# BriansIDP/espnet_slurp

Measured on AMD Instinct MI355X. Metric: utterances/sec (fbank80x1500, Conformer-12L CTC+attn), higher is better.
Workload: dtype f32; 1 GPU; C2 SLURP Conformer-medium d=256 H=4 FF=1024 12L enc / 6L dec, V=600, rel_pos=latest, ctc 0.3, lsm 0.1, dropout 0.1, SpecAug on; global_batch=384, seq_len=1500, parallelism=dp1

## Files before the change

### espnet_slurp_amd/_native.py

```python
from __future__ import annotations

import ctypes
import os

_HERE = os.path.dirname(os.path.abspath(__file__))
LIB_PATH = os.path.join(_HERE, "libespnet_mi355%s.so" % os.environ.get("ESP_LIB_VARIANT", ""))

P = ctypes.c_void_p
I = ctypes.c_int
L = ctypes.c_long
F = ctypes.c_float
U64 = ctypes.c_ulonglong

SIGNATURES = {
    "esp_last_error": [],
    "esp_abi_version": [],
    "esp_gemm_bf16": [I, I, I, I, I, I, I, P, L, L, L, P, L, L, L, P, L, L, L, P, F, F, P, I, P, F, U64, I, P, P, P, L,
                      P],
    "esp_gemm_bf16_pl": [I, I, I, I, I, I, I, P, L, L, L, P, L, L, L, P, L, L, L, P, F, F, I, P, F, U64, I, P, I,
                         L, P, L, P],
    "esp_f32_to_bf16": [P, P, L, I, L, L, I, P],
    "esp_conv2_fwd_bf16": [P, P, P, P, I, I, I, I, P, L, P],
    "esp_conv2_dgrad_bf16": [P, P, P, P, I, I, I, I, P, P, L, P],
    "esp_conv1_fwd_bf16": [P, P, P, P, P, I, I, I, I, P],
# ... 43 lines not shown
    "esp_csgu_bwd_norm": [P, P, P, P, P, P, L, I, P, I, I, I, P, P],
    "esp_bn_swish_fwd": [P, P, P, P, P, P, P, P, F, F, I, I, P, L, I, P, P],
    "esp_bn_swish_eval": [P, P, P, P, P, P, F, I, I, P, P, P],
    "esp_bn_swish_fwd_planes": [P, P, P, P, L, L, I, P, P, P, P, F, F, I, I, P, L, I, P, P],
    "esp_bn_swish_bwd": [P, P, P, P, P, P, P, P, P, I, I, P, L, P, I, P, P],
    "esp_heads_split": [P, L, I, I, I, I, I, P, P, P],
    "esp_heads_split2": [P, L, I, I, I, I, I, P, P, P, P, P],
    "esp_add2d": [P, L, P, L, I, I, P],
    "esp_attn_softmax_fwd": [P, P, I, I, F, P, I, I, P, P, F, U64, I, I, I, L, L, P, P],
    "esp_attn_softmax_bwd": [P, P, P, F, U64, F, L, I, L, P],
    "esp_relshift_bwd": [P, L, P, L, I, I, I, I, P],
    "esp_relpos_attn_fwd": [P, P, P, L, P, L, I, I, F, P, P, P, F, U64, I, L, P],
    "esp_relpos_attn_probs": [P, P, P, L, P, L, I, I, I, F, P, P, P, F, U64, I, L, P, P],
    "esp_attn_bwd_prep": [P, L, P, L, I, I, I, I, P, P, L, I, P],
    "esp_attn_dscores": [P, L, P, L, P, P, P, P, L, I, I, I, I, F, F, U64, I, L, P],
    "esp_attn_softmax_bwd_relpos": [P, P, P, P, L, I, F, U64, F, L, I, L, P, P],
    "esp_attn_softmax_bwd_relpos_band": [P, P, P, P, L, F, U64, F, L, I, L, P],
    "esp_relpos_dqv": [P, L, P, L, P, L, I, I, I, P, L, P],
    "esp_relpos_dq": [P, L, P, L, P, L, P, L, P, I, I, I, P],
    "esp_relpos_attn_bwd": [P, L, P, L, P, P, P, L, I, I, F, F, U64, I, L, P],
    "esp_relpos_flash_fwd": [P, P, P, L, P, L, P, L, I, I, I, F, P, P, L, P, F, U64, I, P],
    "esp_relpos_flash_bwd": [P, P, P, L, P, L, P, L, I, I, I, F, P, P, P, L, P, F, U64, I, P, L, P, P, L, P, P, P],
    "esp_relpos_dp": [P, L, P, I, I, I, I, P, L, P, P, P, P, P, L, P, L, P],
    "esp_fbank_fwd": [P, L, P, I, I, I, I, P, P, P, P, P, I, P, I, P, P],
    "esp_global_mvn": [P, P, I, I, I, P, P, I, I, P],
    "esp_conv2_dgrad": [P, P, P, P, I, I, I, I, P, P, L, P],
    "esp_conv1_fwd": [P, P, P, P, I, I, I, I, P],
    "esp_conv1_fwd_bits": [P, P, P, P, P, P, I, I, I, I, P],
    "esp_conv2_dgrad_bits": [P, P, P, P, P, I, I, I, I, P, P, L, P],
    "esp_conv2_dgrad_c1fold": [P, P, P, P, P, I, I, P, P, I, I, I, I, P, P, L, P, L, P],
# ... 28 lines not shown
    "esp_cbt_unchunk_bwd": [P, P, I, I, I, I, I, I, I, P],
    "esp_conv1_dgrad": [P, P, P, I, I, I, I, P],
    "esp_grad_norm_workspace_bytes": [L],
    "esp_layernorm_bwd_workspace_bytes": [I, I],
    "esp_colsum_workspace_bytes": [I, I],
    "esp_dwconv1d_wgrad_workspace_bytes": [I, I, I, I],
    "esp_bn_swish_fwd_workspace_bytes": [I, I],
    "esp_bn_swish_bwd_workspace_bytes": [I, I],
    "esp_conv1_wgrad_workspace_bytes": [I, I, I, I],
    "esp_conv2_dgrad_workspace_bytes": [I],
    "esp_ctc_loss_workspace_bytes": [I, I, I],
    "esp_relpos_dp_workspace_bytes": [I, I, I],
}
_RESTYPES = {"esp_last_error": ctypes.c_char_p, "esp_abi_version": I, "esp_attn_slot_check_errors": I, "esp_set_gemm_compute": I,
             "esp_get_gemm_compute": I, "esp_set_splitk_mode": I, "esp_set_wgrad_ws": I,
             "esp_f32_gemm_products": I}
_RESTYPES.update({k: L for k in SIGNATURES if k.endswith("_workspace_bytes")})
ABI_VERSION = 39

_lib = None


def load() -> ctypes.CDLL:
    global _lib
    if _lib is not None:
        return _lib
    if not os.path.exists(LIB_PATH):
        raise RuntimeError(
            f"espnet_slurp_amd: native library not found at {LIB_PATH}; "
            "build it with `make -C espnet_slurp_amd/csrc` (no CPU fallback exists)")
    lib = ctypes.CDLL(LIB_PATH)
    for name, args in SIGNATURES.items():
        fn = getattr(lib, name)
# ... 28 lines not shown
```

### espnet_slurp_amd/blocks.py

```python
from __future__ import annotations

import math
from typing import List, Optional

import torch
from torch import nn

from . import kernels as K


def _mix64(x: int) -> int:
    x &= 0xFFFFFFFFFFFFFFFF
    x = ((x ^ (x >> 30)) * 0xBF58476D1CE4E5B9) & 0xFFFFFFFFFFFFFFFF
    x = ((x ^ (x >> 27)) * 0x94D049BB133111EB) & 0xFFFFFFFFFFFFFFFF
    return x ^ (x >> 31)


class Seeds:

    def __init__(self, base: int):
        self.base = base & 0xFFFFFFFFFFFFFFFF
        self.i = 0

    def next(self) -> int:
# ... 273 lines not shown
                   batch=Z, nb2=B, sa=(B * T * Pp, T * Pp), sb=(dk, 0), sc=(dk, T * D))
        K.colsum(tmp, self.pos_bias_v.grad.view(-1), accumulate=True)
        K.add2d(tmp, D, dqkv, 3 * D, M, D)
        dp = empty(P, D, like=dctx)
        K.gemm(P, dk, B * T, dbd, c.q_v, dp, mode_a=K.RC, lda=Pp, mode_b=K.RC, ldb=dk, ldc=D,
               batch=H, nb2=1, sa=(B * T * Pp, 0), sb=(B * T * dk, 0), sc=(dk, 0))
        return dp

    def _bwd_ds(self, c, dctx, dqkv):
        H, dk = self.h, self.d_k
        D = H * dk
        B, T, P = c.B, c.T, c.P
        Z = H * B
        Tp = K.pitch(T)
        dS = empty(Z * T * Tp, like=dctx)
        dot = empty(Z * T, like=dctx)
        K.attn_bwd_prep(dctx, D, c.ctx, D, B, H, dk, T, dot, None, 0, 1)
        K.attn_dscores(dctx, D, c.qkv, 3 * D, c.attn, dot, dS, None, 0, 1, B, H, dk, math.sqrt(dk), c.pa, c.sa, T,
                       Tp, v_off=2 * D)
        self._dv(c, c.pv, dctx, dqkv)
        bias_part = empty(Z * ((T + 31) // 32) * 2 * dk, like=dctx)
        K.relpos_dq(dS, Tp, c.qkv, 3 * D, c.p, D, dqkv, 3 * D, bias_part, B, H, T, k_off=D)
        self._dk(c, dS, dqkv)
        dp = empty(P, D, like=dctx)
        K.relpos_dp(dS, Tp, c.q_v, 1, B, H, T, dp, D, bias_part, None, self.pos_bias_u.grad.view(-1),
                    self.pos_bias_v.grad.view(-1), dqkv, 3 * D)
        return dp

    def _bwd_flash(self, c, dctx, dqkv):
        H, dk = self.h, self.d_k
        D = H * dk
        B, T, P = c.B, c.T, c.P
        Z = H * B
        rel = 2 if self.legacy else 1
# ... 467 lines not shown
```

### espnet_slurp_amd/csrc/attention.hip

```cpp
#include <stdlib.h>

#include <type_traits>

#include "common.h"

namespace {

constexpr int RP_ROWS = 32, RP_DK = 64;

__global__ void heads_split_kernel(const float* __restrict__ src, long ld, int col0, int B, int T, int H, int dk,
                                   const float* __restrict__ bias, float* __restrict__ dst) {
  const long n = (long)H * B * T * dk;
  for (long i = blockIdx.x * (long)blockDim.x + threadIdx.x; i < n; i += (long)gridDim.x * blockDim.x) {
    const int d = (int)(i % dk);
    long r = i / dk;
    const int t = (int)(r % T);
    r /= T;
    const int b = (int)(r % B);
    const int h = (int)(r / B);
    float v = src[((long)b * T + t) * ld + col0 + h * dk + d];
    if (bias) v += bias[h * dk + d];
    dst[i] = v;
  }
}
// ... 660 lines not shown
  for (int t = 0; t < NTA; ++t) {
    const int j = (wave + 4 * t) * 32 + l32;
    if (j >= T) continue;
#pragma unroll
    for (int r = 0; r < 16; ++r) {
      const int i = i0 + (r & 3) + 8 * (r >> 2) + 4 * hf;
      if (i >= T) continue;
      const long row = (long)z * T + i;
      const float pe = sc[t][r] * sm[r];
      attn[row * lds + j] = pe;
      if (pdrop) pdrop[row * lds + j] = esp::keep_elem(seed, (uint64_t)(row * T + j), thr) ? pe * dscale : 0.f;
    }
  }
}

typedef __attribute__((ext_vector_type(8))) __bf16 attn_bf16x8;
struct Frag16 {
  attn_bf16x8 v[2];
};
__device__ __forceinline__ void split_frag(const float (&f)[16], Frag16& o) {
#pragma unroll
  for (int m = 0; m < 2; ++m) {
    uint32_t h[4];
#pragma unroll
    for (int j = 0; j < 4; ++j) h[j] = esp::bf16_pair(f[8 * m + 2 * j], f[8 * m + 2 * j + 1]);
    o.v[m] = __builtin_bit_cast(attn_bf16x8, make_uint4(h[0], h[1], h[2], h[3]));
  }
}
__device__ __forceinline__ f32x4 mfma_np(const Frag16& a, const Frag16& b, f32x4 c) {
#pragma unroll
  for (int m = 0; m < 2; ++m) c = __builtin_amdgcn_mfma_f32_16x16x32_bf16(a.v[m], b.v[m], c, 0, 0, 0);
  return c;
}

#ifndef ESP_ATTN_PROBS_LDS
#define ESP_ATTN_PROBS_LDS 1
#endif
#ifndef ESP_ATTN_PREFETCH
#define ESP_ATTN_PREFETCH 3
#endif

constexpr int RW_ROWS = 16, RW_PITCH = 37;
constexpr int RW_SPITCH = 64;
__device__ __forceinline__ void keep_quad(uint64_t seed, uint64_t ix, uint32_t thr, bool even_T, bool idx32, bool& k0,
                                          bool& k1, bool& k2, bool& k3) {
  if (even_T && idx32) {
    esp::keep_pair32(seed, (uint32_t)ix, thr, k0, k1);
    esp::keep_pair32(seed, (uint32_t)ix + 2, thr, k2, k3);
  } else if (even_T) {
    esp::keep_pair(seed, ix, thr, k0, k1);
    esp::keep_pair(seed, ix + 2, thr, k2, k3);
  } else {
    k0 = esp::keep_elem(seed, ix, thr);
    k1 = esp::keep_elem(seed, ix + 1, thr);
    k2 = esp::keep_elem(seed, ix + 2, thr);
    k3 = esp::keep_elem(seed, ix + 3, thr);
  }
}
template <int NTA, bool P2, bool LEGACY, int SPLIT = 1, int XS = 0>
__global__ __launch_bounds__(256, 2) void relpos_attn_fwd16_kernel(
    const float* __restrict__ qu, const float* __restrict__ qv, const float* __restrict__ kmat, long ldk,
    const float* __restrict__ pm, long ldpm, int nb, float sqrt_dk, const int* __restrict__ klen,
    float* __restrict__ attn, float* __restrict__ pdrop, uint32_t thr, float dscale, uint64_t seed, int T, long lds,
    const uint64_t* __restrict__ key, const int* __restrict__ tvalid, int nrb, int Z) {
  __shared__ float ring[4][RW_ROWS * RW_PITCH];
  __shared__ __attribute__((aligned(16))) float stage[4][RW_ROWS * RW_SPITCH];
  __shared__ float xch[2][4][RW_ROWS];
  const int lane = threadIdx.x & 63, wave = threadIdx.x >> 6;
  const int xcd = blockIdx.x & 7, jb = blockIdx.x >> 3, zq = jb / nrb;
  const int z = zq * 8 + xcd, bx = jb - zq * nrb;
  if (z >= Z) return;
  const int i0 = (SPLIT == 1 ? bx * 4 + wave : bx * 2 + (wave >> 1)) * RW_ROWS;
  const int t0 = SPLIT == 1 ? 0 : (wave & 1) * NTA;
// ... 204 lines not shown
            d.x = k0 ? v.x * dscale : 0.f;
            d.y = k1 ? v.y * dscale : 0.f;
            d.z = k2 ? v.z * dscale : 0.f;
            d.w = k3 ? v.w * dscale : 0.f;
            *reinterpret_cast<float4*>(dbase[ps] + 16 * (t0 + t4)) = d;
          }
        }
      }
      asm volatile("" ::: "memory");
    }
  };
  if (pdrop) store_rows(std::true_type{});
  else store_rows(std::false_type{});
}

__device__ __forceinline__ int swz16(int r) { return ((r >> 1) & 1) | (r & 4); }
template <int NPL>
struct FragPl {
  attn_bf16x8 v[NPL][2];
};
template <int NPL>
__device__ __forceinline__ void split_row16(const float (&f)[16], FragPl<NPL>& o) {
#pragma unroll
  for (int m = 0; m < 2; ++m) {
    uint32_t h[4], md[4], l[4];
#pragma unroll
    for (int j = 0; j < 4; ++j) {
      if constexpr (NPL == 3) esp::split3_pair(f[8 * m + 2 * j], f[8 * m + 2 * j + 1], h[j], md[j], l[j]);
      else h[j] = esp::bf16_pair(f[8 * m + 2 * j], f[8 * m + 2 * j + 1]);
    }
    o.v[0][m] = __builtin_bit_cast(attn_bf16x8, make_uint4(h[0], h[1], h[2], h[3]));
    if constexpr (NPL == 3) {
      o.v[1][m] = __builtin_bit_cast(attn_bf16x8, make_uint4(md[0], md[1], md[2], md[3]));
      o.v[2][m] = __builtin_bit_cast(attn_bf16x8, make_uint4(l[0], l[1], l[2], l[3]));
    }
  }
}
template <int NPL>
__device__ __forceinline__ void read_frag_pl(const uint8_t* tile, int plane_bytes, int li, int q4, FragPl<NPL>& o) {
#pragma unroll
  for (int p = 0; p < NPL; ++p)
#pragma unroll
    for (int m = 0; m < 2; ++m)
      o.v[p][m] = *reinterpret_cast<const attn_bf16x8*>(tile + p * plane_bytes + li * 128 + (((2 * q4 + m) ^ swz16(li)) << 4));
}
template <int NPL>
__device__ __forceinline__ f32x4 mfma_pl(const FragPl<NPL>& a, const FragPl<NPL>& b, f32x4 c) {
#pragma unroll
  for (int m = 0; m < 2; ++m) {
    if constexpr (NPL == 3) {
      c = __builtin_amdgcn_mfma_f32_16x16x32_bf16(a.v[1][m], b.v[1][m], c, 0, 0, 0);
      c = __builtin_amdgcn_mfma_f32_16x16x32_bf16(a.v[2][m], b.v[0][m], c, 0, 0, 0);
      c = __builtin_amdgcn_mfma_f32_16x16x32_bf16(a.v[0][m], b.v[2][m], c, 0, 0, 0);
      c = __builtin_amdgcn_mfma_f32_16x16x32_bf16(a.v[1][m], b.v[0][m], c, 0, 0, 0);
      c = __builtin_amdgcn_mfma_f32_16x16x32_bf16(a.v[0][m], b.v[1][m], c, 0, 0, 0);
    }
    c = __builtin_amdgcn_mfma_f32_16x16x32_bf16(a.v[0][m], b.v[0][m], c, 0, 0, 0);
  }
  return c;
}

#ifndef ESP_ATTN_SLOT_CHECK
#define ESP_ATTN_SLOT_CHECK 0
#endif
#if ESP_ATTN_SLOT_CHECK
__device__ int g_attn_slot_err[64];
#endif
template <int NTA, bool P2, bool LEGACY, int NP>
__global__ __launch_bounds__(256, 2) void relpos_probs_lds_kernel(
    const float* __restrict__ qu, const float* __restrict__ qv, const float* __restrict__ kmat, long ldk,
    const float* __restrict__ pm, long ldpm, int nb, float sqrt_dk, const int* __restrict__ klen,
    float* __restrict__ attn, float* __restrict__ pdrop, uint32_t thr, float dscale, uint64_t seed, int T, long lds,
    const uint64_t* __restrict__ key, const int* __restrict__ tvalid, int nrb, int Z) {
  constexpr int NPL = NP == 6 ? 3 : 1;
  constexpr int PLB = RW_ROWS * 128;
// ... 31 lines not shown
    asm volatile("" ::: "memory");
    bool bad = false;
#pragma unroll
    for (int w = 0; w < 4; ++w) bad |= gw[w] != v;
    asm volatile("" ::: "memory");
    if (bad) g_attn_slot_err[lane] = 1 + where;
  };
#define ESP_SLOT_MARK(g, v) mark(g, v)
#define ESP_SLOT_CHECK(g, v, w) check(g, v, w)
#else
#define ESP_SLOT_MARK(g, v) ((void)0)
#define ESP_SLOT_CHECK(g, v, w) ((void)0)
#endif

  const int sr = tid >> 4, sd = 4 * (tid & 15);
  const int woff = sr * 128 + (((sd >> 3) ^ swz16(sr)) << 4) + ((sd >> 2) & 1) * 8;
  auto k_src = [&](int t) {
    return reinterpret_cast<const float4*>(kmat + ((long)b * T + min(t * 16 + sr, T - 1)) * ldk + head * RP_DK + sd);
  };
  auto p_src = [&](int u) {
    int pos = pbase + 16 * u + sr;
    if (LEGACY && pos > Ts) pos -= Ts + 1;
    return reinterpret_cast<const float4*>(pm + (long)min(max(pos, 0), P - 1) * ldpm + head * RP_DK + sd);
  };
  auto put_tile = [&](uint8_t* dst, const float4 v) {
    if constexpr (NPL == 3) {
      uint32_t h0, m0, l0, h1, m1, l1;
      esp::split3_pair(v.x, v.y, h0, m0, l0);
      esp::split3_pair(v.z, v.w, h1, m1, l1);
      *reinterpret_cast<uint2*>(dst + woff) = make_uint2(h0, h1);
      *reinterpret_cast<uint2*>(dst + PLB + woff) = make_uint2(m0, m1);
      *reinterpret_cast<uint2*>(dst + 2 * PLB + woff) = make_uint2(l0, l1);
    } else {
      *reinterpret_cast<uint2*>(dst + woff) = make_uint2(esp::bf16_pair(v.x, v.y), esp::bf16_pair(v.z, v.w));
    }
  };
  {
    float4 pv[PSL];
#pragma unroll
    for (int s = 0; s < PSL; ++s) pv[s] = *p_src(s - 4);
    const float4 kv = *k_src(0);
#pragma unroll
    for (int s = 0; s < PSL; ++s) {
      ESP_SLOT_MARK(pgen[pslot(s - 4)], BUSY);
      put_tile(ppl[pslot(s - 4)], pv[s]);
      ESP_SLOT_MARK(pgen[pslot(s - 4)], s - 4);
    }
    ESP_SLOT_MARK(kgen[0], BUSY);
    put_tile(kpl[0], kv);
    ESP_SLOT_MARK(kgen[0], 0);
    if constexpr (LEGACY) {
// ... 176 lines not shown
      }
      asm volatile("" ::: "memory");
    }
  };
  if (pdrop) store_rows(std::true_type{});
  else store_rows(std::false_type{});
#undef ESP_SLOT_MARK
#undef ESP_SLOT_CHECK
}

inline int gridn(long n) {
  long b = (n + 255) / 256;
  return (int)(b > 65536 ? 65536 : (b < 1 ? 1 : b));
}

template <int... Cs>
struct IntList {};
template <int C0, int... Cs, class F>
inline void dispatch_ge(IntList<C0, Cs...>, int v, F&& f) {
  if constexpr (sizeof...(Cs) == 0) {
    f(std::integral_constant<int, C0>{});
  } else {
    if (v <= C0) f(std::integral_constant<int, C0>{});
    else dispatch_ge(IntList<Cs...>{}, v, f);
  }
}
template <class F>
inline void dispatch_bool(bool b, F&& f) {
  if (b) f(std::true_type{});
  else f(std::false_type{});
}
struct DropArgs {
  uint32_t thr;
  float scale;
};
inline DropArgs drop_args(float drop_p) {
  const uint32_t thr = esp::drop_threshold(drop_p);
  return {thr, esp::drop_scale(thr)};
}
inline DropArgs drop_args(float drop_p, float*& pdrop) {
  const DropArgs d = drop_args(drop_p);
  if (!d.thr) pdrop = nullptr;
  return d;
}
inline bool is_pow2(float x) { return x > 0.f && (__builtin_bit_cast(uint32_t, x) & 0x7fffffu) == 0; }
using Per64 = IntList<1, 2, 4, 8, 16>;

}

ESP_API int esp_attn_slot_check_errors(void) {
#if ESP_ATTN_SLOT_CHECK
  if (hipDeviceSynchronize() != hipSuccess) return -2;
  int h[64];
  if (hipMemcpyFromSymbol(h, HIP_SYMBOL(g_attn_slot_err), sizeof h) != hipSuccess) return -2;
  int n = 0;
  for (int i = 0; i < 64; ++i) n += h[i] != 0;
  const int zeros[64] = {};
  if (hipMemcpyToSymbol(HIP_SYMBOL(g_attn_slot_err), zeros, sizeof zeros) != hipSuccess) return -2;
  return n;
// ... 295 lines not shown
```

### espnet_slurp_amd/csrc/attention_bwd.hip

```cpp
#include <stdlib.h>

#include "common.h"

namespace {

constexpr int QR = 32, QDK = 64, QKS = 32;
typedef __attribute__((ext_vector_type(8))) __bf16 bf16x8;

__device__ __forceinline__ int il_of(int r, int hf) { return (r & 3) + 8 * (r >> 2) + 4 * hf; }

__device__ __forceinline__ void split8(const float* v, bf16x8 (&o)[3]) {
  uint32_t H[4], M[4], L[4];
#pragma unroll
  for (int p = 0; p < 4; ++p) esp::split3_pair(v[2 * p], v[2 * p + 1], H[p], M[p], L[p]);
  o[0] = __builtin_bit_cast(bf16x8, make_uint4(H[0], H[1], H[2], H[3]));
  o[1] = __builtin_bit_cast(bf16x8, make_uint4(M[0], M[1], M[2], M[3]));
  o[2] = __builtin_bit_cast(bf16x8, make_uint4(L[0], L[1], L[2], L[3]));
}
__device__ __forceinline__ void mma6(f32x16& acc, const bf16x8 (&a)[3], const bf16x8 (&b)[3]) {
  constexpr int PA[6] = {1, 2, 0, 1, 0, 0}, PB[6] = {1, 0, 2, 0, 1, 0};
#pragma unroll
  for (int p = 0; p < 6; ++p) acc = __builtin_amdgcn_mfma_f32_32x32x16_bf16(a[PA[p]], b[PB[p]], acc, 0, 0, 0);
}

// ... 134 lines not shown
  if (job == 1) {
#pragma unroll
    for (int r = 0; r < 16; ++r) vt[(c * QR + il_of(r, hf)) * VP + l32] = acc[r];
  }
  __syncthreads();
  if (job == 0) {
#pragma unroll
    for (int r = 0; r < 16; ++r) {
      const int row = il_of(r, hf);
      if (i0 + row < T)
        dq[((long)b * T + i0 + row) * ldq + QDK * head + 32 * c + l32] = acc[r] + vt[(c * QR + row) * VP + l32];
    }
  }
}

}

static int relpos_dq_pitch(int T) { return (T + 31) / 32 * 32 + 4; }

ESP_API int esp_relpos_dq(const float* dS, long lds, const float* kmat, long ldk, const float* p, long ldpm, float* dq,
                          long ldq, float* bias_part, int nb, int H, int T, void* stream) {
  ESP_ARG_CHECK(T >= 1 && nb >= 1 && H >= 1 && lds >= T && lds % 4 == 0 && ((uintptr_t)dS & 15) == 0,
                "esp_relpos_dq: bad sizes T=%d lds=%ld (lds %% 4 == 0, dS 16-B aligned)", T, lds);
  const int DSP = relpos_dq_pitch(T);
  size_t shm = (size_t)QR * DSP * sizeof(float);
  if (shm < 2 * QR * 33 * sizeof(float)) shm = 2 * QR * 33 * sizeof(float);
  ESP_ARG_CHECK(shm <= 65536 && DSP <= 512, "esp_relpos_dq: T=%d needs %zu B of LDS (T <= 480)", T, shm);
  ESP_ARG_CHECK(dq && bias_part && kmat && p, "esp_relpos_dq: null operand");
  ESP_ARG_CHECK(ldk >= 64 && ldpm >= 64 && ldk < (1L << 22) && ldpm < (1L << 22) && 4L * T * ldk < (1L << 31) &&
                    4L * (2 * T - 1) * ldpm < (1L << 31),
// ... 8 lines not shown
```

### espnet_slurp_amd/csrc/elementwise.hip

```cpp
#include <stdarg.h>
#include <stdio.h>

#include "common.h"

namespace esp {
static thread_local char g_err[512] = "";
static const uint64_t* g_rng_key = nullptr;
const uint64_t* rng_key_ptr() { return g_rng_key; }
void set_error(const char* fmt, ...) {
  va_list ap;
  va_start(ap, fmt);
  vsnprintf(g_err, sizeof(g_err), fmt, ap);
  va_end(ap);
}
}

ESP_API const char* esp_last_error(void) { return esp::g_err; }
ESP_API int esp_abi_version(void) { return 39; }
ESP_API int esp_set_rng_key(const unsigned long long* key) {
  esp::g_rng_key = (const uint64_t*)key;
  return 0;
}

namespace {


inline int grid_for(long n, int per_thread = 1) {
  long b = (n / per_thread + 255) / 256;
  if (b > 65536) b = 65536;
  return (int)(b < 1 ? 1 : b);
}

__global__ void act_bwd_kernel(const float* __restrict__ dy, const float* __restrict__ h,
// ... 552 lines not shown
```

### espnet_slurp_amd/kernels.py

```python
from __future__ import annotations

import math
import os
from typing import Optional, Sequence

import torch

from . import _native

KC, RC, I2C_KC, I2C_RC = 0, 1, 2, 3
ACT_NONE, ACT_RELU, ACT_SWISH = 0, 1, 2
ACT_MUL = 3
ACT_AUX_DERIV = 16


def _p(t: Optional[torch.Tensor], off: int = 0):
    if t is None:
        return None
    return t.data_ptr() + off * t.element_size()


def _st():
    return torch.cuda.current_stream().cuda_stream

# ... 699 lines not shown
    lib = _native.load()
    prev = lib.esp_set_splitk_mode(int(mode))
    if prev < 0:
        raise _native.NativeError(f"esp_set_splitk_mode failed: {lib.esp_last_error().decode()}")
    return prev


def set_wgrad_ws(mode: int) -> int:
    lib = _native.load()
    prev = lib.esp_set_wgrad_ws(int(mode))
    if prev < 0:
        raise _native.NativeError(f"esp_set_wgrad_ws failed: {lib.esp_last_error().decode()}")
    return prev


def get_gemm_compute() -> int:
    return _native.load().esp_get_gemm_compute()


class gemm_compute:

    def __init__(self, dtype):
        self.dtype = dtype

    def __enter__(self):
        self.prev = set_gemm_compute(self.dtype)
        return self

    def __exit__(self, *exc):
        set_gemm_compute(self.prev)
# ... 185 lines not shown
def attn_dscores(dctx, ldd, vmat, ldv, attn, dot, dS, dbd, ldp, relpos, nb, H, dk, sqrt_dk, drop_p, seed, T, lds,
                 v_off=0):
    _f32(dctx, vmat, attn, dot, dS, dbd)
    if _PROF is not None:
        ev0 = torch.cuda.Event(enable_timing=True)
        ev1 = torch.cuda.Event(enable_timing=True)
        ev0.record()
    _native.call("esp_attn_dscores", _p(dctx), ldd, _p(vmat, v_off), ldv, _p(attn), _p(dot), _p(dS), _p(dbd), ldp,
                 int(relpos), nb, H, dk, float(sqrt_dk), float(drop_p), int(seed) & (2 ** 64 - 1), T, lds, _st())
    if _PROF is not None:
        ev1.record()
        _PROF.append((2.0 * T * T * dk * nb * H, ev0, ev1, (KC, KC, T, T, dk, nb * H, "dscores"),
                      (8.0 if dbd is not None else 4.0) * T * T * nb * H))


FLASH_ATTN = False
ATTN_FWD32 = False
FUSED_ATTN_BWD = False
ATTN_DSCORES = False
RELPOS_BWD_DS = True


def flash_ok(T: int, dk: int) -> bool:
    return FLASH_ATTN and dk == 64 and 1 <= T <= 512


def relpos_probs_ok(T: int, dk: int) -> bool:
    return dk == 64 and T <= 512


def relpos_fused_ok(T: int, dk: int) -> bool:
    return dk == 64 and (32 * (32 * ((T + 62) // 32) + 4) + 256) * 4 <= 65536


def relpos_bwd_ds_ok(T: int, dk: int) -> bool:
    return dk == 64 and 1 <= T <= 480 and pitch(T) % 4 == 0


def relpos_attn_paths(T: int, dk: int, legacy: bool, bucketed: bool):
    if flash_ok(T, dk) and not bucketed:
        fwd = "flash"
    elif relpos_probs_ok(T, dk) and not ATTN_FWD32:
        fwd = "probs"
    elif not legacy and relpos_fused_ok(T, dk):
        fwd = "block32"
    else:
        fwd = "gemm"
    if fwd == "flash":
        bwd = "flash"
    elif (not legacy and RELPOS_BWD_DS and relpos_bwd_ds_ok(T, dk) and not FUSED_ATTN_BWD and not ATTN_DSCORES
          and _COMPUTE[0] == GEMM_FP32):
# ... 534 lines not shown
```

### include/espnet_mi355.h

```cpp
#ifndef ESPNET_MI355_H
#define ESPNET_MI355_H
#ifdef __cplusplus
extern "C" {
#endif

const char* esp_last_error(void);
int esp_abi_version(void);

int esp_gemm_f32(int mode_a, int mode_b, int M, int N, int K, int batch, int nb2,
                 const float* A, long lda, long sa1, long sa2,
                 const float* B, long ldb, long sb1, long sb2,
                 float* C, long ldc, long sc1, long sc2,
                 const float* bias, float alpha, float beta, const float* R,
                 int act, float* aux, float drop_p, unsigned long long seed,
                 int bwd_act, const float* pre, float* rowsum,
                 const int* im2col_a, const int* im2col_b, float* work, long work_bytes,
                 void* stream);
int esp_set_gemm_compute(int dtype);
int esp_get_gemm_compute(void);
int esp_f32_gemm_products(void);
int esp_set_splitk_mode(int mode);
int esp_set_wgrad_ws(int mode);
int esp_gemm_f32_bp(int mode_a, int mode_b, int M, int N, int K, int batch, int nb2, const float* A, long lda,
                    long sa1, long sa2, const float* B, long ldb, long sb1, long sb2, float* C, long ldc,
// ... 139 lines not shown
                         float* pdrop, long lds, float* bias_part, float* carry, void* stream);
int esp_relpos_dp(const float* dS, long lds, const float* qv, int rel, int nb, int H, int T, float* dp, long ldp,
                  const float* bias_part, const float* carry, float* du, float* dv, float* dq, long ldq,
                  float* work, long work_floats, void* stream);
int esp_relpos_dq(const float* dS, long lds, const float* kmat, long ldk, const float* p, long ldpm, float* dq,
                  long ldq, float* bias_part, int nb, int H, int T, void* stream);
int esp_relpos_attn_fwd(const float* qu, const float* qv, const float* kmat, long ldk, const float* p,
                        long ldp_row, int nb, int H, float sqrt_dk, const int* klen, float* attn,
                        float* pdrop, float drop_p, unsigned long long seed, int T, long lds,
                        void* stream);
int esp_attn_bwd_prep(const float* dctx, long ldd, const float* ctx, long ldc, int nb, int H, int dk, int T,
                      float* dot, float* dbd, long ldp, int relpos, void* stream);
int esp_attn_dscores(const float* dctx, long ldd, const float* vmat, long ldv, const float* attn, const float* dot,
                     float* dS, float* dbd, long ldp, int relpos, int nb, int H, int dk, float sqrt_dk,
                     float drop_p, unsigned long long seed, int T, long lds, void* stream);
int esp_attn_slot_check_errors(void);
int esp_relpos_attn_probs(const float* qu, const float* qv, const float* kmat, long ldk, const float* p,
                          long ldp_row, int relpos, int nb, int H, float sqrt_dk, const int* klen,
                          float* attn, float* pdrop, float drop_p, unsigned long long seed, int T,
                          long lds, const int* tvalid, void* stream);

int esp_fbank_fwd(const float* wave, long ldw, const int* lens, int B, int N, int n_fft, int hop,
                  const float* window, const float* twiddle, const float* melw, const int* mel_lo,
                  const int* mel_hi, int n_mels, float* out, int T, const int* nvalid, void* stream);
int esp_global_mvn(float* x, const int* lens, int B, int T, int F, const float* mean,
                   const float* stdv, int norm_means, int norm_vars, void* stream);

int esp_conv1_fwd(const float* x, const float* W, const float* bias, float* z, int B, int T,
                  int F, int D, void* stream);
int esp_conv1_fwd_bf16(const float* x, const float* W, const float* bias, float* z, void* z16, int B, int T, int F,
// ... 93 lines not shown
```

Before: 1547 utt/s.

## Fuse relpos attention backward prep and dscores into one MFMA kernel

Adds a relpos_dscores kernel that computes the row dot(dctx, ctx), the dV-projection dP = dctx·Vᵀ via split-bf16 (3-plane) MFMA, dropout masking and the softmax backward in a single pass writing dS. It replaces the separate attn_bwd_prep and attn_dscores launches in the _bwd_ds path when T<=480 and dk=64. Shared tile helpers move into a new attn_tiles.h header. The 3-plane bf16 split is meant to keep near-f32 accuracy while using matrix cores, at the cost of extra MFMA work and LDS usage.

```diff
diff --git a/espnet_slurp_amd/_native.py b/espnet_slurp_amd/_native.py
--- a/espnet_slurp_amd/_native.py
+++ b/espnet_slurp_amd/_native.py
@@ -81,6 +81,9 @@
     "esp_relpos_attn_probs": [P, P, P, L, P, L, I, I, I, F, P, P, P, F, U64, I, L, P, P],
     "esp_attn_bwd_prep": [P, L, P, L, I, I, I, I, P, P, L, I, P],
     "esp_attn_dscores": [P, L, P, L, P, P, P, P, L, I, I, I, I, F, F, U64, I, L, P],
+    "esp_set_relpos_dscores": [I],
+    "esp_relpos_dscores_on": [I, I],
+    "esp_relpos_dscores": [P, L, P, L, P, L, P, P, L, I, I, F, F, U64, I, P],
     "esp_attn_softmax_bwd_relpos": [P, P, P, P, L, I, F, U64, F, L, I, L, P, P],
     "esp_attn_softmax_bwd_relpos_band": [P, P, P, P, L, F, U64, F, L, I, L, P],
     "esp_relpos_dqv": [P, L, P, L, P, L, I, I, I, P, L, P],
@@ -139,9 +142,9 @@
 }
 _RESTYPES = {"esp_last_error": ctypes.c_char_p, "esp_abi_version": I, "esp_attn_slot_check_errors": I, "esp_set_gemm_compute": I,
              "esp_get_gemm_compute": I, "esp_set_splitk_mode": I, "esp_set_wgrad_ws": I,
-             "esp_f32_gemm_products": I}
+             "esp_f32_gemm_products": I, "esp_set_relpos_dscores": I, "esp_relpos_dscores_on": I}
 _RESTYPES.update({k: L for k in SIGNATURES if k.endswith("_workspace_bytes")})
-ABI_VERSION = 39
+ABI_VERSION = 40
 
 _lib = None
 
diff --git a/espnet_slurp_amd/blocks.py b/espnet_slurp_amd/blocks.py
--- a/espnet_slurp_amd/blocks.py
+++ b/espnet_slurp_amd/blocks.py
@@ -311,10 +311,14 @@
         Z = H * B
         Tp = K.pitch(T)
         dS = empty(Z * T * Tp, like=dctx)
-        dot = empty(Z * T, like=dctx)
-        K.attn_bwd_prep(dctx, D, c.ctx, D, B, H, dk, T, dot, None, 0, 1)
-        K.attn_dscores(dctx, D, c.qkv, 3 * D, c.attn, dot, dS, None, 0, 1, B, H, dk, math.sqrt(dk), c.pa, c.sa, T,
-                       Tp, v_off=2 * D)
+        if K.relpos_dscores_ok(T, dk):
+            K.relpos_dscores(dctx, D, c.ctx, D, c.qkv, 3 * D, c.attn, dS, Tp, B, H, math.sqrt(dk), c.pa, c.sa, T,
+                             v_off=2 * D)
+        else:
+            dot = empty(Z * T, like=dctx)
+            K.attn_bwd_prep(dctx, D, c.ctx, D, B, H, dk, T, dot, None, 0, 1)
+            K.attn_dscores(dctx, D, c.qkv, 3 * D, c.attn, dot, dS, None, 0, 1, B, H, dk, math.sqrt(dk), c.pa, c.sa,
+                           T, Tp, v_off=2 * D)
         self._dv(c, c.pv, dctx, dqkv)
         bias_part = empty(Z * ((T + 31) // 32) * 2 * dk, like=dctx)
         K.relpos_dq(dS, Tp, c.qkv, 3 * D, c.p, D, dqkv, 3 * D, bias_part, B, H, T, k_off=D)
diff --git a/espnet_slurp_amd/csrc/attention.hip b/espnet_slurp_amd/csrc/attention.hip
--- a/espnet_slurp_amd/csrc/attention.hip
+++ b/espnet_slurp_amd/csrc/attention.hip
@@ -2,7 +2,10 @@
 
 #include <type_traits>
 
+#include "attn_tiles.h"
 #include "common.h"
+
+using namespace esp::attn;
 
 namespace {
 
@@ -698,7 +701,6 @@
   }
 }
 
-typedef __attribute__((ext_vector_type(8))) __bf16 attn_bf16x8;
 struct Frag16 {
   attn_bf16x8 v[2];
 };
@@ -726,21 +728,6 @@
 
 constexpr int RW_ROWS = 16, RW_PITCH = 37;
 constexpr int RW_SPITCH = 64;
-__device__ __forceinline__ void keep_quad(uint64_t seed, uint64_t ix, uint32_t thr, bool even_T, bool idx32, bool& k0,
-                                          bool& k1, bool& k2, bool& k3) {
-  if (even_T && idx32) {
-    esp::keep_pair32(seed, (uint32_t)ix, thr, k0, k1);
-    esp::keep_pair32(seed, (uint32_t)ix + 2, thr, k2, k3);
-  } else if (even_T) {
-    esp::keep_pair(seed, ix, thr, k0, k1);
-    esp::keep_pair(seed, ix + 2, thr, k2, k3);
-  } else {
-    k0 = esp::keep_elem(seed, ix, thr);
-    k1 = esp::keep_elem(seed, ix + 1, thr);
-    k2 = esp::keep_elem(seed, ix + 2, thr);
-    k3 = esp::keep_elem(seed, ix + 3, thr);
-  }
-}
 template <int NTA, bool P2, bool LEGACY, int SPLIT = 1, int XS = 0>
 __global__ __launch_bounds__(256, 2) void relpos_attn_fwd16_kernel(
     const float* __restrict__ qu, const float* __restrict__ qv, const float* __restrict__ kmat, long ldk,
@@ -975,51 +962,6 @@
   else store_rows(std::false_type{});
 }
 
-__device__ __forceinline__ int swz16(int r) { return ((r >> 1) & 1) | (r & 4); }
-template <int NPL>
-struct FragPl {
-  attn_bf16x8 v[NPL][2];
-};
-template <int NPL>
-__device__ __forceinline__ void split_row16(const float (&f)[16], FragPl<NPL>& o) {
-#pragma unroll
-  for (int m = 0; m < 2; ++m) {
-    uint32_t h[4], md[4], l[4];
-#pragma unroll
-    for (int j = 0; j < 4; ++j) {
-      if constexpr (NPL == 3) esp::split3_pair(f[8 * m + 2 * j], f[8 * m + 2 * j + 1], h[j], md[j], l[j]);
-      else h[j] = esp::bf16_pair(f[8 * m + 2 * j], f[8 * m + 2 * j + 1]);
-    }
-    o.v[0][m] = __builtin_bit_cast(attn_bf16x8, make_uint4(h[0], h[1], h[2], h[3]));
-    if constexpr (NPL == 3) {
-      o.v[1][m] = __builtin_bit_cast(attn_bf16x8, make_uint4(md[0], md[1], md[2], md[3]));
-      o.v[2][m] = __builtin_bit_cast(attn_bf16x8, make_uint4(l[0], l[1], l[2], l[3]));
-    }
-  }
-}
-template <int NPL>
-__device__ __forceinline__ void read_frag_pl(const uint8_t* tile, int plane_bytes, int li, int q4, FragPl<NPL>& o) {
-#pragma unroll
-  for (int p = 0; p < NPL; ++p)
-#pragma unroll
-    for (int m = 0; m < 2; ++m)
-      o.v[p][m] = *reinterpret_cast<const attn_bf16x8*>(tile + p * plane_bytes + li * 128 + (((2 * q4 + m) ^ swz16(li)) << 4));
-}
-template <int NPL>
-__device__ __forceinline__ f32x4 mfma_pl(const FragPl<NPL>& a, const FragPl<NPL>& b, f32x4 c) {
-#pragma unroll
-  for (int m = 0; m < 2; ++m) {
-    if constexpr (NPL == 3) {
-      c = __builtin_amdgcn_mfma_f32_16x16x32_bf16(a.v[1][m], b.v[1][m], c, 0, 0, 0);
-      c = __builtin_amdgcn_mfma_f32_16x16x32_bf16(a.v[2][m], b.v[0][m], c, 0, 0, 0);
-      c = __builtin_amdgcn_mfma_f32_16x16x32_bf16(a.v[0][m], b.v[2][m], c, 0, 0, 0);
-      c = __builtin_amdgcn_mfma_f32_16x16x32_bf16(a.v[1][m], b.v[0][m], c, 0, 0, 0);
-      c = __builtin_amdgcn_mfma_f32_16x16x32_bf16(a.v[0][m], b.v[1][m], c, 0, 0, 0);
-    }
-    c = __builtin_amdgcn_mfma_f32_16x16x32_bf16(a.v[0][m], b.v[0][m], c, 0, 0, 0);
-  }
-  return c;
-}
 
 #ifndef ESP_ATTN_SLOT_CHECK
 #define ESP_ATTN_SLOT_CHECK 0
@@ -1081,7 +1023,7 @@
 #endif
 
   const int sr = tid >> 4, sd = 4 * (tid & 15);
-  const int woff = sr * 128 + (((sd >> 3) ^ swz16(sr)) << 4) + ((sd >> 2) & 1) * 8;
+  const int woff = tile_woff(sr, sd);
   auto k_src = [&](int t) {
     return reinterpret_cast<const float4*>(kmat + ((long)b * T + min(t * 16 + sr, T - 1)) * ldk + head * RP_DK + sd);
   };
@@ -1090,18 +1032,7 @@
     if (LEGACY && pos > Ts) pos -= Ts + 1;
     return reinterpret_cast<const float4*>(pm + (long)min(max(pos, 0), P - 1) * ldpm + head * RP_DK + sd);
   };
-  auto put_tile = [&](uint8_t* dst, const float4 v) {
-    if constexpr (NPL == 3) {
-      uint32_t h0, m0, l0, h1, m1, l1;
-      esp::split3_pair(v.x, v.y, h0, m0, l0);
-      esp::split3_pair(v.z, v.w, h1, m1, l1);
-      *reinterpret_cast<uint2*>(dst + woff) = make_uint2(h0, h1);
-      *reinterpret_cast<uint2*>(dst + PLB + woff) = make_uint2(m0, m1);
-      *reinterpret_cast<uint2*>(dst + 2 * PLB + woff) = make_uint2(l0, l1);
-    } else {
-      *reinterpret_cast<uint2*>(dst + woff) = make_uint2(esp::bf16_pair(v.x, v.y), esp::bf16_pair(v.z, v.w));
-    }
-  };
+  auto put_tile = [&](uint8_t* dst, const float4 v) { put_tile_pl<NPL>(dst, PLB, woff, v); };
   {
     float4 pv[PSL];
 #pragma unroll
@@ -1308,35 +1239,6 @@
   return (int)(b > 65536 ? 65536 : (b < 1 ? 1 : b));
 }
 
-template <int... Cs>
-struct IntList {};
-template <int C0, int... Cs, class F>
-inline void dispatch_ge(IntList<C0, Cs...>, int v, F&& f) {
-  if constexpr (sizeof...(Cs) == 0) {
-    f(std::integral_constant<int, C0>{});
-  } else {
-    if (v <= C0) f(std::integral_constant<int, C0>{});
-    else dispatch_ge(IntList<Cs...>{}, v, f);
-  }
-}
-template <class F>
-inline void dispatch_bool(bool b, F&& f) {
-  if (b) f(std::true_type{});
-  else f(std::false_type{});
-}
-struct DropArgs {
-  uint32_t thr;
-  float scale;
-};
-inline DropArgs drop_args(float drop_p) {
-  const uint32_t thr = esp::drop_threshold(drop_p);
-  return {thr, esp::drop_scale(thr)};
-}
-inline DropArgs drop_args(float drop_p, float*& pdrop) {
-  const DropArgs d = drop_args(drop_p);
-  if (!d.thr) pdrop = nullptr;
-  return d;
-}
 inline bool is_pow2(float x) { return x > 0.f && (__builtin_bit_cast(uint32_t, x) & 0x7fffffu) == 0; }
 using Per64 = IntList<1, 2, 4, 8, 16>;
 
diff --git a/espnet_slurp_amd/csrc/attention_bwd.hip b/espnet_slurp_amd/csrc/attention_bwd.hip
--- a/espnet_slurp_amd/csrc/attention_bwd.hip
+++ b/espnet_slurp_amd/csrc/attention_bwd.hip
@@ -1,6 +1,9 @@
 #include <stdlib.h>
 
+#include "attn_tiles.h"
 #include "common.h"
+
+using namespace esp::attn;
 
 namespace {
 
@@ -172,6 +175,184 @@
   }
 }
 
+#ifndef ESP_RELPOS_DSCORES
+#define ESP_RELPOS_DSCORES 1
+#endif
+#ifndef ESP_DSCORES_VPF
+#define ESP_DSCORES_VPF 4
+#endif
+int g_relpos_dscores = 1;
+
+#if ESP_RELPOS_DSCORES
+constexpr int DS_ROWS = 16, DS_TMAX = 480;
+template <bool DROP>
+__global__ __launch_bounds__(256, 3) void relpos_dscores_kernel(
+    const float* __restrict__ dctx, long ldd, const float* __restrict__ ctx, long ldc, const float* __restrict__ vmat,
+    long ldv, const float* __restrict__ attn, float* __restrict__ dS, long lds, int nb, float alpha, uint32_t thr,
+    float dscale, uint64_t seed, const uint64_t* __restrict__ key, int T, int nrb, int Z) {
+  constexpr int PLB = DS_ROWS * 128;
+  constexpr int GT = 4;
+  constexpr int VPF = ESP_DSCORES_VPF;
+  static_assert(GT % 2 == 0 && GT % VPF == 0, "the LDS slot and the V prefetch slot of a tile are fixed per unrolled step");
+  __shared__ __attribute__((aligned(16))) uint8_t vpl[2][3 * PLB];
+  __shared__ __attribute__((aligned(16))) float stage[4][DS_ROWS * 16 * GT];
+  __shared__ float dotl[4][DS_ROWS];
+  const int tid = threadIdx.x, lane = tid & 63, wave = __builtin_amdgcn_readfirstlane(tid >> 6);
+  const int xcd = blockIdx.x & 7, jb = blockIdx.x >> 3, zq = jb / nrb;
+  const int z = zq * 8 + xcd, bx = jb - zq * nrb;
+  if (z >= Z) return;
+  const int i0 = bx * 4 * DS_ROWS + wave * DS_ROWS;
+  seed = esp::keyed(seed, key);
+  const int head = z / nb, b = z - head * nb;
+  const int li = lane & 15, q4 = lane >> 4;
+  const int ng = (T + 16 * GT - 1) / (16 * GT);
+
+  const int sr = tid >> 4, sd = 4 * (tid & 15);
+  const int woff = tile_woff(sr, sd);
+  const float* vbase = vmat + (long)b * T * ldv + head * QDK + sd;
+  auto v_src = [&](int t) { return reinterpret_cast<const float4*>(vbase + (long)min(t * DS_ROWS + sr, T - 1) * ldv); };
+  float4 nv[VPF];
+  const float4 v0 = *v_src(0);
+#pragma unroll
+  for (int s = 1; s <= VPF; ++s) nv[s % VPF] = *v_src(s);
+
+  const int rs = q4, c = li;
+  const int jmax = (T - 1) & ~3;
+  long roff[4];
+  bool rok[4];
+#pragma unroll
+  for (int ps = 0; ps < 4; ++ps) {
+    const int i = i0 + 4 * ps + rs;
+    rok[ps] = i < T;
+    roff[ps] = ((long)z * T + min(i, T - 1)) * lds;
+  }
+  auto p_ld = [&](int ps, int g) {
+    return *reinterpret_cast<const float4*>(attn + roff[ps] + min(16 * GT * g + 4 * c, jmax));
+  };
+  float4 pq[4];
+#pragma unroll
+  for (int ps = 0; ps < 4; ++ps) pq[ps] = p_ld(ps, 0);
+
+  FragPl<3> xd;
+  float dotr[4];
+  {
+    const long row = (long)b * T + min(i0 + li, T - 1);
+    float f[16], x[16];
+    const float4* g4 = reinterpret_cast<const float4*>(dctx + row * ldd + head * QDK + 16 * q4);
+    const float4* c4 = reinterpret_cast<const float4*>(ctx + row * ldc + head * QDK + 16 * q4);
+#pragma unroll
+    for (int u = 0; u < 4; ++u) {
+      const float4 g = g4[u], y = c4[u];
+      f[4 * u] = g.x; f[4 * u + 1] = g.y; f[4 * u + 2] = g.z; f[4 * u + 3] = g.w;
+      x[4 * u] = y.x; x[4 * u + 1] = y.y; x[4 * u + 2] = y.z; x[4 * u + 3] = y.w;
+    }
+    float s4[4];
+#pragma unroll
+    for (int u = 0; u < 4; ++u)
+      s4[u] = f[4 * u] * x[4 * u] + f[4 * u + 1] * x[4 * u + 1] + f[4 * u + 2] * x[4 * u + 2] + f[4 * u + 3] * x[4 * u + 3];
+    float dot = (s4[0] + s4[1]) + (s4[2] + s4[3]);
+    dot += __shfl_xor(dot, 16, 64);
+    dot += __shfl_xor(dot, 32, 64);
+    split_row16(f, xd);
+    if (q4 == 0) dotl[wave][li] = dot;
+    asm volatile("" ::: "memory");
+#pragma unroll
+    for (int ps = 0; ps < 4; ++ps) dotr[ps] = dotl[wave][4 * ps + rs];
+  }
+  put_tile_pl<3>(vpl[0], PLB, woff, v0);
+  const bool even_T = (T & 1) == 0;
+  const bool idx32 = (uint64_t)Z * (uint64_t)T * (uint64_t)T <= 0xffffffffull;
+  const uint64_t ib0 = ((uint64_t)z * (uint64_t)T + (uint64_t)(i0 + rs)) * (uint64_t)T + (uint64_t)(4 * c);
+  float* stg = stage[wave];
+  __syncthreads();
+
+#pragma unroll 1
+  for (int g = 0; g < ng; ++g) {
+#pragma unroll
+    for (int u = 0; u < GT; ++u) {
+      const int t = GT * g + u;
+      FragPl<3> vf;
+      read_frag_pl(vpl[u & 1], PLB, li, q4, vf);
+      *reinterpret_cast<f32x4*>(stg + li * (16 * GT) + (((4 * u + q4) ^ li) << 2)) =
+          mfma_pl(vf, xd, f32x4{0.f, 0.f, 0.f, 0.f});
+      put_tile_pl<3>(vpl[(u + 1) & 1], PLB, woff, nv[(u + 1) % VPF]);
+      nv[(u + 1) % VPF] = *v_src(t + 1 + VPF);
+      __syncthreads();
+    }
+    asm volatile("" ::: "memory");
+    f32x4 dp[4];
+#pragma unroll
+    for (int ps = 0; ps < 4; ++ps)
+      dp[ps] = *reinterpret_cast<const f32x4*>(stg + (4 * ps + rs) * (16 * GT) + ((c ^ (4 * ps + rs)) << 2));
+    asm volatile("" ::: "memory");
+    const int j = 16 * GT * g + 4 * c;
+#pragma unroll
+    for (int ps = 0; ps < 4; ++ps) {
+      if (rok[ps] && j < T) {
+        bool k0 = true, k1 = true, k2 = true, k3 = true;
+        if (DROP)
+          keep_quad(seed, ib0 + (uint64_t)(4 * ps) * (uint64_t)T + (uint64_t)(16 * GT * g), thr, even_T, idx32, k0, k1, k2, k3);
+        const float4 p = pq[ps];
+        const float dot = dotr[ps];
+        float4 o;
+        o.x = p.x * ((k0 ? (DROP ? dp[ps][0] * dscale : dp[ps][0]) : 0.f) - dot) * alpha;
+        o.y = p.y * ((k1 ? (DROP ? dp[ps][1] * dscale : dp[ps][1]) : 0.f) - dot) * alpha;
+        o.z = p.z * ((k2 ? (DROP ? dp[ps][2] * dscale : dp[ps][2]) : 0.f) - dot) * alpha;
+        o.w = p.w * ((k3 ? (DROP ? dp[ps][3] * dscale : dp[ps][3]) : 0.f) - dot) * alpha;
+        *reinterpret_cast<float4*>(dS + roff[ps] + j) = o;
+      }
+    }
+#pragma unroll
+    for (int ps = 0; ps < 4; ++ps) pq[ps] = p_ld(ps, g + 1);
+  }
+}
+#endif
+
+}
+
+ESP_API int esp_set_relpos_dscores(int mode) {
+  ESP_ARG_CHECK(mode >= 0 && mode <= 2, "esp_set_relpos_dscores: mode must be 0, 1 or 2, got %d", mode);
+  const int prev = g_relpos_dscores;
+  g_relpos_dscores = mode;
+  return prev;
+}
+
+ESP_API int esp_relpos_dscores_on(int T, int dk) {
+#if ESP_RELPOS_DSCORES
+  return g_relpos_dscores != 0 && dk == QDK && T >= 1 && T <= DS_TMAX;
+#else
+  return 0;
+#endif
+}
+
+ESP_API int esp_relpos_dscores(const float* dctx, long ldd, const float* ctx, long ldc, const float* vmat, long ldv,
+                               const float* attn, float* dS, long lds, int nb, int H, float sqrt_dk, float drop_p,
+                               unsigned long long seed, int T, void* stream) {
+#if ESP_RELPOS_DSCORES
+  ESP_ARG_CHECK(T >= 1 && T <= DS_TMAX && nb >= 1 && H >= 1 && lds >= T && lds % 4 == 0 && sqrt_dk > 0.f,
+                "esp_relpos_dscores: bad sizes T=%d lds=%ld (1 <= T <= 480, lds %% 4 == 0)", T, lds);
+  ESP_ARG_CHECK(dctx && ctx && vmat && attn && dS, "esp_relpos_dscores: null operand");
+  ESP_ARG_CHECK(((uintptr_t)attn & 15) == 0 && ((uintptr_t)dS & 15) == 0, "esp_relpos_dscores: attn / dS not 16-B aligned");
+  ESP_ARG_CHECK(ldd % 4 == 0 && ldc % 4 == 0 && ldv % 4 == 0 && ldd >= (long)QDK * H && ldc >= (long)QDK * H &&
+                    ldv >= (long)QDK * H && ((uintptr_t)dctx & 15) == 0 && ((uintptr_t)ctx & 15) == 0 &&
+                    ((uintptr_t)vmat & 15) == 0,
+                "esp_relpos_dscores: dctx / ctx / V must be 16-B aligned with ld %% 4 == 0 and ld >= 64 H");
+  ESP_ARG_CHECK(drop_p >= 0.f && drop_p < 1.f, "dropout p must be in [0, 1) (got %g)", (double)drop_p);
+  const DropArgs dr = drop_args(drop_p);
+  const int Z = nb * H;
+  const int nrb = (T + 4 * DS_ROWS - 1) / (4 * DS_ROWS);
+  const dim3 grid((unsigned)(8 * ((Z + 7) / 8) * nrb));
+  dispatch_bool(dr.thr != 0, [&](auto drop) {
+    hipLaunchKernelGGL(relpos_dscores_kernel<decltype(drop)::value>, grid, dim3(256), 0, (hipStream_t)stream, dctx, ldd,
+                       ctx, ldc, vmat, ldv, attn, dS, lds, nb, 1.0f / sqrt_dk, dr.thr, dr.scale, (uint64_t)seed,
+                       esp::rng_key_ptr(), T, nrb, Z);
+  });
+  ESP_CHECK_LAUNCH("esp_relpos_dscores");
+  return 0;
+#else
+  esp::set_error("esp_relpos_dscores: not in this build (ESP_RELPOS_DSCORES=0)");
+  return -1;
+#endif
 }
 
 static int relpos_dq_pitch(int T) { return (T + 31) / 32 * 32 + 4; }
diff --git a/espnet_slurp_amd/csrc/attn_tiles.h b/espnet_slurp_amd/csrc/attn_tiles.h
--- /dev/null
+++ b/espnet_slurp_amd/csrc/attn_tiles.h
@@ -0,0 +1,120 @@
+#pragma once
+#include <type_traits>
+
+#include "common.h"
+
+namespace esp {
+namespace attn {
+
+typedef __attribute__((ext_vector_type(8))) __bf16 attn_bf16x8;
+
+__device__ __forceinline__ void keep_quad(uint64_t seed, uint64_t ix, uint32_t thr, bool even_T, bool idx32, bool& k0,
+                                          bool& k1, bool& k2, bool& k3) {
+  if (even_T && idx32) {
+    esp::keep_pair32(seed, (uint32_t)ix, thr, k0, k1);
+    esp::keep_pair32(seed, (uint32_t)ix + 2, thr, k2, k3);
+  } else if (even_T) {
+    esp::keep_pair(seed, ix, thr, k0, k1);
+    esp::keep_pair(seed, ix + 2, thr, k2, k3);
+  } else {
+    k0 = esp::keep_elem(seed, ix, thr);
+    k1 = esp::keep_elem(seed, ix + 1, thr);
+    k2 = esp::keep_elem(seed, ix + 2, thr);
+    k3 = esp::keep_elem(seed, ix + 3, thr);
+  }
+}
+
+__device__ __forceinline__ int swz16(int r) { return ((r >> 1) & 1) | (r & 4); }
+template <int NPL>
+struct FragPl {
+  attn_bf16x8 v[NPL][2];
+};
+template <int NPL>
+__device__ __forceinline__ void split_row16(const float (&f)[16], FragPl<NPL>& o) {
+#pragma unroll
+  for (int m = 0; m < 2; ++m) {
+    uint32_t h[4], md[4], l[4];
+#pragma unroll
+    for (int j = 0; j < 4; ++j) {
+      if constexpr (NPL == 3) esp::split3_pair(f[8 * m + 2 * j], f[8 * m + 2 * j + 1], h[j], md[j], l[j]);
+      else h[j] = esp::bf16_pair(f[8 * m + 2 * j], f[8 * m + 2 * j + 1]);
+    }
+    o.v[0][m] = __builtin_bit_cast(attn_bf16x8, make_uint4(h[0], h[1], h[2], h[3]));
+    if constexpr (NPL == 3) {
+      o.v[1][m] = __builtin_bit_cast(attn_bf16x8, make_uint4(md[0], md[1], md[2], md[3]));
+      o.v[2][m] = __builtin_bit_cast(attn_bf16x8, make_uint4(l[0], l[1], l[2], l[3]));
+    }
+  }
+}
+__device__ __forceinline__ int tile_woff(int sr, int sd) {
+  return sr * 128 + (((sd >> 3) ^ swz16(sr)) << 4) + ((sd >> 2) & 1) * 8;
+}
+template <int NPL>
+__device__ __forceinline__ void put_tile_pl(uint8_t* dst, int plane_bytes, int woff, const float4 v) {
+  if constexpr (NPL == 3) {
+    uint32_t h0, m0, l0, h1, m1, l1;
+    esp::split3_pair(v.x, v.y, h0, m0, l0);
+    esp::split3_pair(v.z, v.w, h1, m1, l1);
+    *reinterpret_cast<uint2*>(dst + woff) = make_uint2(h0, h1);
+    *reinterpret_cast<uint2*>(dst + plane_bytes + woff) = make_uint2(m0, m1);
+    *reinterpret_cast<uint2*>(dst + 2 * plane_bytes + woff) = make_uint2(l0, l1);
+  } else {
+    *reinterpret_cast<uint2*>(dst + woff) = make_uint2(esp::bf16_pair(v.x, v.y), esp::bf16_pair(v.z, v.w));
+  }
+}
+template <int NPL>
+__device__ __forceinline__ void read_frag_pl(const uint8_t* tile, int plane_bytes, int li, int q4, FragPl<NPL>& o) {
+#pragma unroll
+  for (int p = 0; p < NPL; ++p)
+#pragma unroll
+    for (int m = 0; m < 2; ++m)
+      o.v[p][m] = *reinterpret_cast<const attn_bf16x8*>(tile + p * plane_bytes + li * 128 + (((2 * q4 + m) ^ swz16(li)) << 4));
+}
+template <int NPL>
+__device__ __forceinline__ f32x4 mfma_pl(const FragPl<NPL>& a, const FragPl<NPL>& b, f32x4 c) {
+#pragma unroll
+  for (int m = 0; m < 2; ++m) {
+    if constexpr (NPL == 3) {
+      c = __builtin_amdgcn_mfma_f32_16x16x32_bf16(a.v[1][m], b.v[1][m], c, 0, 0, 0);
+      c = __builtin_amdgcn_mfma_f32_16x16x32_bf16(a.v[2][m], b.v[0][m], c, 0, 0, 0);
+      c = __builtin_amdgcn_mfma_f32_16x16x32_bf16(a.v[0][m], b.v[2][m], c, 0, 0, 0);
+      c = __builtin_amdgcn_mfma_f32_16x16x32_bf16(a.v[1][m], b.v[0][m], c, 0, 0, 0);
+      c = __builtin_amdgcn_mfma_f32_16x16x32_bf16(a.v[0][m], b.v[1][m], c, 0, 0, 0);
+    }
+    c = __builtin_amdgcn_mfma_f32_16x16x32_bf16(a.v[0][m], b.v[0][m], c, 0, 0, 0);
+  }
+  return c;
+}
+
+template <int... Cs>
+struct IntList {};
+template <int C0, int... Cs, class F>
+inline void dispatch_ge(IntList<C0, Cs...>, int v, F&& f) {
+  if constexpr (sizeof...(Cs) == 0) {
+    f(std::integral_constant<int, C0>{});
+  } else {
+    if (v <= C0) f(std::integral_constant<int, C0>{});
+    else dispatch_ge(IntList<Cs...>{}, v, f);
+  }
+}
+template <class F>
+inline void dispatch_bool(bool b, F&& f) {
+  if (b) f(std::true_type{});
+  else f(std::false_type{});
+}
+struct DropArgs {
+  uint32_t thr;
+  float scale;
+};
+inline DropArgs drop_args(float drop_p) {
+  const uint32_t thr = esp::drop_threshold(drop_p);
+  return {thr, esp::drop_scale(thr)};
+}
+inline DropArgs drop_args(float drop_p, float*& pdrop) {
+  const DropArgs d = drop_args(drop_p);
+  if (!d.thr) pdrop = nullptr;
+  return d;
+}
+
+}
+}
diff --git a/espnet_slurp_amd/csrc/elementwise.hip b/espnet_slurp_amd/csrc/elementwise.hip
--- a/espnet_slurp_amd/csrc/elementwise.hip
+++ b/espnet_slurp_amd/csrc/elementwise.hip
@@ -16,7 +16,7 @@
 }
 
 ESP_API const char* esp_last_error(void) { return esp::g_err; }
-ESP_API int esp_abi_version(void) { return 39; }
+ESP_API int esp_abi_version(void) { return 40; }
 ESP_API int esp_set_rng_key(const unsigned long long* key) {
   esp::g_rng_key = (const uint64_t*)key;
   return 0;
diff --git a/espnet_slurp_amd/kernels.py b/espnet_slurp_amd/kernels.py
--- a/espnet_slurp_amd/kernels.py
+++ b/espnet_slurp_amd/kernels.py
@@ -737,6 +737,14 @@
     return prev
 
 
+def set_relpos_dscores(mode: int) -> int:
+    lib = _native.load()
+    prev = lib.esp_set_relpos_dscores(int(mode))
+    if prev < 0:
+        raise _native.NativeError(f"esp_set_relpos_dscores failed: {lib.esp_last_error().decode()}")
+    return prev
+
+
 def get_gemm_compute() -> int:
     return _native.load().esp_get_gemm_compute()
 
@@ -952,6 +960,12 @@
                       (8.0 if dbd is not None else 4.0) * T * T * nb * H))
 
 
+def relpos_dscores(dctx, ldd, ctx, ldc, vmat, ldv, attn, dS, lds, nb, H, sqrt_dk, drop_p, seed, T, v_off=0):
+    _f32(dctx, ctx, vmat, attn, dS)
+    _native.call("esp_relpos_dscores", _p(dctx), ldd, _p(ctx), ldc, _p(vmat, v_off), ldv, _p(attn), _p(dS), lds, nb,
+                 H, float(sqrt_dk), float(drop_p), int(seed) & (2 ** 64 - 1), T, _st())
+
+
 FLASH_ATTN = False
 ATTN_FWD32 = False
 FUSED_ATTN_BWD = False
@@ -973,6 +987,10 @@
 
 def relpos_bwd_ds_ok(T: int, dk: int) -> bool:
     return dk == 64 and 1 <= T <= 480 and pitch(T) % 4 == 0
+
+
+def relpos_dscores_ok(T: int, dk: int) -> bool:
+    return relpos_bwd_ds_ok(T, dk) and bool(_native.load().esp_relpos_dscores_on(int(T), int(dk)))
 
 
 def relpos_attn_paths(T: int, dk: int, legacy: bool, bucketed: bool):
diff --git a/include/espnet_mi355.h b/include/espnet_mi355.h
--- a/include/espnet_mi355.h
+++ b/include/espnet_mi355.h
@@ -177,6 +177,11 @@
 int esp_attn_dscores(const float* dctx, long ldd, const float* vmat, long ldv, const float* attn, const float* dot,
                      float* dS, float* dbd, long ldp, int relpos, int nb, int H, int dk, float sqrt_dk,
                      float drop_p, unsigned long long seed, int T, long lds, void* stream);
+int esp_set_relpos_dscores(int mode);
+int esp_relpos_dscores_on(int T, int dk);
+int esp_relpos_dscores(const float* dctx, long ldd, const float* ctx, long ldc, const float* vmat, long ldv,
+                       const float* attn, float* dS, long lds, int nb, int H, float sqrt_dk, float drop_p,
+                       unsigned long long seed, int T, void* stream);
 int esp_attn_slot_check_errors(void);
 int esp_relpos_attn_probs(const float* qu, const float* qv, const float* kmat, long ldk, const float* p,
                           long ldp_row, int relpos, int nb, int H, float sqrt_dk, const int* klen,
```

Result: no change. 1561 utt/s (median of 6 runs) (+0.9%).
